# apple/foundationdb

Hardware: AMD Instinct MI355X
Metric: device-resident CRC32C GiB/s on 4 KiB page batches; % of HBM-read peak (higher is better)
Workload: dtype u8; 1 GPU; 1048576 x 4096 B pages, device-resident, fixed stride; pages=1048576, page_bytes=4096, seed=0, stride=4096

## Files before the change

foundationdb_amd/csrc/crc32c_device.h:

```cpp
#pragma once
#include <stdint.h>
#include <hip/hip_runtime.h>

#include <mutex>

namespace fdbcrc {

constexpr uint32_t kV7TabSlots = 64u;

struct DevTables {
	uint32_t slice[2][256];
	uint32_t block[8][16];
	uint32_t lane[64][8][16];
	uint32_t slice4[4][256];
	uint32_t inv_z[16][8][16];
	uint32_t pow2[64][8][16];
	uint32_t corr[4][16][8][16];
	uint32_t table_shift[8][16];
	uint32_t slotw[64][16][8][16];
	uint32_t carryw[64][16][8][16];
	uint32_t chunkpow[256][8][16];
	uint32_t bpow[4][256][8][16];
	uint32_t xinv64[65][8][16];
	uint32_t pow64[64][8][16];
	uint32_t pow1[64][8][16];
	uint32_t stride4[4][256];
	uint32_t lane_s[64][8][16];
};

void build_dev_tables(DevTables* t);

constexpr uint32_t kPageCtrWords = 32;

#ifndef FDBCRC_XCD_EVEN_W
#define FDBCRC_XCD_EVEN_W 33
#define FDBCRC_XCD_ODD_W 31
#endif
constexpr uint64_t kXcdEvenW = FDBCRC_XCD_EVEN_W, kXcdOddW = FDBCRC_XCD_ODD_W;
struct XcdRanges {
	uint64_t n, pe, po;
	__device__ __forceinline__ XcdRanges(uint64_t n_, uint64_t G) : n(n_) {
		const uint64_t ne = (G + 1) / 2, no = G / 2;
		const uint64_t den = ne * kXcdEvenW + no * kXcdOddW;
		const uint64_t unit = (n * 32 + den - 1) / den;
		pe = (unit * kXcdEvenW + 31) / 32;
		po = (unit * kXcdOddW + 31) / 32;
	}
	__device__ __forceinline__ void get(uint64_t b, uint64_t& g0, uint64_t& g1) const {
		const uint64_t s0 = ((b + 1) / 2) * pe + (b / 2) * po;
		const uint64_t e0 = s0 + ((b & 1) ? po : pe);
		g0 = s0 < n ? s0 : n;
		g1 = e0 < n ? e0 : n;
	}
};
__device__ __forceinline__ void xcd_range(uint64_t n, uint64_t b, uint64_t G, uint64_t& g0, uint64_t& g1) {
	XcdRanges(n, G).get(b, g0, g1);
}
int page_counters(hipStream_t stream, int num_cus, uint32_t** ctr);
constexpr uint64_t kAuxBytes = 256;
constexpr int kAuxPktFrames = 0;
constexpr int kAuxPageCtr = 8;
int stream_aux(hipStream_t stream, uint64_t** aux, std::unique_lock<std::mutex>* hold = nullptr);

int launch_pages(int blocks_per_page, const uint8_t* base, uint64_t stride, uint64_t count, uint32_t seed,
                 const uint32_t* seeds, uint32_t* out, const DevTables* tabs, int num_cus, hipStream_t stream);
int launch_pages_window(const uint8_t* pages, uint64_t stride, uint64_t count, uint32_t h, uint32_t t, uint32_t seed,
                        const uint32_t* seeds, uint32_t* out, const DevTables* tabs, int num_cus, hipStream_t stream);
int launch_pages_window_list(const uint8_t* pages, uint64_t stride, const uint32_t* idx, const uint64_t* d_count,
                             uint64_t max_count, uint32_t h, uint32_t t, uint32_t seed, uint32_t* out,
                             const DevTables* tabs, int num_cus, hipStream_t stream);
enum : int { kRouteBoth = 0, kRouteWindows = 1, kRouteBlocks = 2, kRouteExtent = 3 };
constexpr int kHstatNblk = 3, kHstatPacked = 4, kHstatXfail = 5;
constexpr uint64_t kXfailBackoff = 16;
inline int route_for_stats(const volatile uint64_t* s) {
	const uint64_t win = s[0], mid = s[1], large = s[2];
	const bool big = large != 0 && large >= win + mid;
	if (s[kHstatPacked] == 1 && s[kHstatXfail] == 0 && !big) return kRouteExtent;
	if (!big) return kRouteWindows;
	return win == 0 ? kRouteBlocks : kRouteBoth;
}
constexpr uint64_t kXMaxExtent = 1ull << 40;
#ifndef FDBX_GRAB_MIN
#define FDBX_GRAB_MIN 8
#endif
constexpr uint64_t kXGrabMin = FDBX_GRAB_MIN;
static_assert(kXGrabMin >= 8 && (kXGrabMin & (kXGrabMin - 1)) == 0, "grabs: a power of two of at least 8 blocks");
__host__ __device__ inline uint64_t x_gsz(uint64_t nblk, uint64_t capg) {
	uint64_t gsz = kXGrabMin;
	while (capg && (nblk + gsz - 1) / gsz > capg) gsz <<= 1;
	return gsz;
}
__host__ __device__ inline uint32_t x_log2(uint64_t v) {
	uint32_t l = 0;
	while ((1ull << l) < v) ++l;
	return l;
}
constexpr uint64_t kXGrabCap = 1ull << 18;
constexpr int kXStage = 8;
struct XState {
	uint32_t* xhdr;
	uint32_t* ps;
	uint32_t* pe;
	uint32_t* dummy;
	uint32_t* ragg;
	uint32_t* wq;
	uint32_t* gagg;
	uint64_t capg;
	uint32_t* ctr;
	uint32_t epoch;
};
uint64_t extent_state_bytes(uint64_t count, uint64_t capg, int num_cus);
void extent_state_carve(void* mem, uint64_t count, uint64_t capg, int num_cus, XState* x);
uint64_t varlen_workspace_bytes(uint64_t count, uint64_t nwave);
int launch_varlen(const uint8_t* base, const uint64_t* offsets, const uint64_t* lengths, uint64_t count, uint32_t seed,
                  const uint32_t* seeds, uint32_t* out, const DevTables* tabs, int num_cus, void* ws,
                  hipStream_t stream, int route = kRouteBoth, uint64_t* hstat = nullptr, uint32_t* err = nullptr,
                  const XState* xs = nullptr, uint32_t* bacc = nullptr, uint32_t* pctr = nullptr);
inline const uint64_t* varlen_refused_word(const void* ws) { return static_cast<const uint64_t*>(ws) + 6; }
int launch_fixed_general(const uint8_t* base, uint64_t stride, uint64_t length, uint64_t count, uint32_t seed,
                         const uint32_t* seeds, uint32_t* out, const DevTables* tabs, int num_cus, void* ws,
                         hipStream_t stream);
uint64_t varlen7_workspace_bytes(uint64_t count, uint64_t nwave);
int launch_varlen7(const uint8_t* base, const uint64_t* offsets, const uint64_t* lengths, uint64_t stride,
                   uint64_t length, uint64_t count, uint32_t seed, const uint32_t* seeds, uint32_t* out,
                   const DevTables* tabs, int num_cus, void* ws, hipStream_t stream, int route, uint64_t* hstat,
                   uint32_t* err = nullptr, const XState* xs = nullptr, uint32_t* bacc = nullptr,
                   uint32_t* pctr = nullptr);
int launch_extent(const uint8_t* base, const uint64_t* offsets, const uint64_t* lengths, uint64_t stride,
                  uint64_t length, uint64_t count, uint32_t seed, const uint32_t* seeds, uint32_t* out,
                  const DevTables* tabs, int num_cus, const XState& xs, uint64_t* hstat, hipStream_t stream,
                  int phase);
int launch_chain_fold(const uint64_t* starts, uint64_t nchains, const uint64_t* lengths, const uint32_t* segcrc,
                      uint32_t seed, const uint32_t* seeds, uint32_t* out, const DevTables* tabs, int num_cus,
                      hipStream_t stream);
struct BigEnt {
	uint64_t E;
	uint32_t s;
	uint32_t idx;
	uint32_t lot;
	uint32_t sd;
};
struct BigParams {
	const uint64_t* hdr;
	const BigEnt* ent;
	uint32_t* out;
	uint32_t* ctr;
	const DevTables* tabs;
	const uint8_t* base;
	const uint64_t* offsets;
	const uint64_t* lengths;
	uint64_t nbuf;
	uint32_t seed;
	const uint32_t* seeds;
	uint32_t* acc;
	BigEnt* priv;
	uint64_t* hstat;
	uint32_t* err;
};
constexpr uint64_t kNPMax = 6144;
constexpr uint64_t kNPAccBytes = 8 * kNPMax + 32;
int launch_bigblocks_np(const BigParams& P, int num_cus, hipStream_t stream);
constexpr uint64_t kBigMax = 1ull << 40;
int launch_bigblocks(const BigParams& P, int num_cus, hipStream_t stream);
int launch_fill_seeds(uint64_t count, uint32_t seed, const uint32_t* seeds, uint32_t* out, hipStream_t stream);

}
```

foundationdb_amd/csrc/crc32c_kernels.hip:

```cpp

#include <hip/hip_runtime.h>
#include <stdint.h>

#include <type_traits>

#include "crc32c_common.h"

#ifndef FDBCRC_PU
#define FDBCRC_PU 2
#endif

namespace fdbcrc {

template <int U, bool WINDOW, bool RAW = WINDOW>
__device__ __forceinline__ void unit_crc_b(const uint32_t* lds, int lane, uint32_t c4, uint32_t c_lane,
                                           Block (&u)[U], const uint32_t (&s)[U], uint32_t (&crc)[U],
                                           uint32_t h, uint32_t t) {
	if (WINDOW) {
#pragma unroll
		for (int j = 0; j < U; ++j) {
			const Masks mk = edge_masks(h, 16 - t, ~s[j]);
#pragma unroll
			for (int d = 0; d < 4; ++d) {
				const uint32_t m0 = lane == 0 ? mk.lm[d] : ~0u;
				const uint32_t x0 = lane == 0 ? mk.inj[d] : ((d == 0 && lane == 32) ? mk.spill : 0u);
				u[j].r[0][d] = (u[j].r[0][d] & m0) ^ x0;
				u[j].r[3][d] &= lane == 63 ? mk.tm[d] : ~0u;
			}
		}
	}
#pragma unroll
	for (int j = 0; j < U; ++j) unswizzle(u[j]);
	uint32_t x[U];
#pragma unroll
	for (int j = 0; j < U; ++j) x[j] = (!WINDOW && lane == 0) ? ~s[j] : 0u;
#pragma unroll
	for (int j = 0; j < U; ++j) x[j] ^= u[j].r[0][0];
#pragma unroll
	for (int w = 0; w < 16; ++w)
#pragma unroll
		for (int j = 0; j < U; ++j) x[j] = word_step4_next(lds, x[j], w < 15 ? u[j].r[(w + 1) >> 2][(w + 1) & 3] : 0u, c4);
#pragma unroll
	for (int j = 0; j < U; ++j) {
		const uint32_t r = wave_xor(mul_nibbles(lds, x[j], c_lane));
		crc[j] = RAW ? r : ~r;
	}
}

struct BlockS {
	uint32_t w[16];
};
typedef __attribute__((address_space(1))) const uint32_t g_u32k;
__device__ __forceinline__ void load_block_s(BlockS& b, const uint8_t* page, uint32_t lane4) {
	const uint8_t* p = page + lane4;
#pragma unroll
	for (int k = 0; k < 16; ++k) b.w[k] = __builtin_nontemporal_load((g_u32k*)reinterpret_cast<uintptr_t>(p + 256 * k));
}
template <int U, bool WINDOW, bool RAW = WINDOW>
__device__ __forceinline__ void unit_crc_s(const uint32_t* lds, int lane, uint32_t c4, uint32_t c_lane,
                                           BlockS (&u)[U], const uint32_t (&s)[U], uint32_t (&crc)[U],
                                           uint32_t h, uint32_t t) {
	uint32_t x[U];
	if (WINDOW) {
		const int d = (int)h - 4 * lane;
		const uint32_t keep0 = d <= 0 ? ~0u : (d >= 4 ? 0u : ~0u << (8 * d));
		const int cut = 256 - (int)t - 4 * lane;
		const uint32_t keep15 = cut >= 4 ? ~0u : (cut <= 0 ? 0u : ~0u >> (8 * (4 - cut)));
#pragma unroll
		for (int j = 0; j < U; ++j) {
			const uint32_t sd = ~s[j];
			const uint32_t inj = (d > -4 && d < 4) ? (d >= 0 ? sd << (8 * d) : sd >> (-8 * d)) : 0u;
			x[j] = (u[j].w[0] & keep0) ^ inj;
			u[j].w[15] &= keep15;
		}
	} else {
#pragma unroll
		for (int j = 0; j < U; ++j) x[j] = (lane == 0 ? ~s[j] : 0u) ^ u[j].w[0];
	}
#pragma unroll
	for (int w = 0; w < 16; ++w)
#pragma unroll
		for (int j = 0; j < U; ++j) x[j] = word_step4_next(lds, x[j], w < 15 ? u[j].w[w + 1] : 0u, c4);
#pragma unroll
	for (int j = 0; j < U; ++j) {
		const uint32_t r = wave_xor(mul_nibbles(lds, x[j], c_lane));
		crc[j] = RAW ? r : ~r;
	}
}

__device__ __forceinline__ uint32_t vmul_tab(const uint32_t (*tab)[16], uint32_t v) {
	typedef __attribute__((address_space(1))) const uint32_t g_u32;
	uint32_t r = 0;
#pragma unroll
	for (int n = 0; n < 8; ++n)
		r ^= *((g_u32*)reinterpret_cast<uintptr_t>(&tab[n][(v >> (4 * n)) & 15u]));
	return r;
}

#ifdef FDBCRC_BTIMES
__device__ uint64_t g_bt[16384][4];
__device__ uint64_t g_bt2[16384][4];
#define FDBCRC_BT2(k) \
	{ \
		const uint64_t tk = __builtin_amdgcn_s_memrealtime(); \
		const uint32_t wk = blockIdx.x * 16 + (threadIdx.x >> 6); \
		if ((threadIdx.x & 63) == 0) __hip_atomic_store(&g_bt2[wk][k], tk, __ATOMIC_RELAXED, __HIP_MEMORY_SCOPE_AGENT); \
	}
#else
#define FDBCRC_BT2(k)
#endif
#ifndef FDBCRC_STRIDED
#define FDBCRC_STRIDED 0
#endif
template <int U, bool WINDOW = false, bool LIST = false, bool PAIR = false, bool STRIDED = FDBCRC_STRIDED>
__global__ __launch_bounds__(1024) void k_pages4k(const uint8_t* __restrict__ base, uint64_t stride, uint64_t count,
                                                  uint32_t seed, const uint32_t* __restrict__ seeds,
                                                  uint32_t* __restrict__ out, const DevTables* __restrict__ tabs,
                                                  uint32_t* __restrict__ ctr, uint32_t h = 0, uint32_t t = 0,
                                                  const uint32_t* __restrict__ idx = nullptr,
                                                  const uint64_t* __restrict__ d_count = nullptr) {
	if (LIST) {
		count = *d_count;
		if (count == 0) return;
	}
	if (PAIR) count *= 2;
#ifdef FDBCRC_BTIMES
	const uint64_t pt0 = __builtin_amdgcn_s_memrealtime();
#endif
	constexpr uint32_t C = 2 * U;
	constexpr uint32_t F = 64 / C;
	static_assert(64 % C == 0, "a store group fills the wave's lanes");
	__shared__ uint32_t lds[kLdsBytesB / 4];
	const LaneCtx c = make_ctx();
	const uint32_t col4 = (c.lane & 31) * 4;
	const uint32_t c4 = col4 | 0x10000u;
	const uint32_t c_lane = (kS4LaneOff + (c.lane >> 5) * 0x4000) | col4;
	const uint32_t wpb = blockDim.x >> 6;
	const uint32_t wi = rdfirst(threadIdx.x >> 6);
	const uint64_t ngrab = (count + C - 1) / C;
	uint64_t g0, g1;
	xcd_range(ngrab, blockIdx.x, gridDim.x, g0, g1);
	uint32_t* const my_ctr = ctr + kPageCtrWords * blockIdx.x;
	const uint64_t last = count - 1;
	auto page = [&](uint64_t i) {
		const uint64_t j = i < count ? i : last;
		if (PAIR) return base + (j >> 1) * stride + (j & 1) * 4096;
		return base + (LIST ? (uint64_t)idx[j] : j) * stride;
	};
	typedef typename std::conditional<STRIDED, BlockS, Block>::type Blk;
	const uint32_t lane4 = 4u * (uint32_t)c.lane;
	auto load_u = [&](Blk (&u)[U], uint64_t i0) {
#pragma unroll
		for (int j = 0; j < U; ++j) {
			if constexpr (STRIDED)
				load_block_s(u[j], page(i0 + j), lane4);
			else
				load_block(u[j], page(i0 + j), c.ld_off);
		}
	};
	auto unit = [&](Blk (&u)[U], const uint32_t (&sd)[U], uint32_t (&crc)[U]) {
		if constexpr (STRIDED)
			unit_crc_s<U, WINDOW, WINDOW || PAIR>(lds, c.lane, c4, c_lane, u, sd, crc, h, t);
		else
			unit_crc_b<U, WINDOW, WINDOW || PAIR>(lds, c.lane, c4, c_lane, u, sd, crc, h, t);
	};
	auto clampg = [&](uint64_t g) { return g < g1 ? g : ngrab; };
	auto request = [&]() -> uint32_t {
		uint32_t r = 0;
		if (c.lane == 0) r = atomicAdd(my_ctr, 1u);
		return r;
	};
	auto seed_of = [&](uint64_t g) -> uint32_t {
		const uint64_t i = g * C + (uint64_t)(c.lane & (C - 1));
		const uint64_t j = i < count ? i : last;
		const uint32_t v = *(seeds ? seeds + (PAIR ? j >> 1 : j) : &tabs->slice4[0][0]);
		const uint32_t sd = seeds ? v : seed;
		return (PAIR && (c.lane & 1)) ? ~0u : sd;
	};
	uint64_t gA = clampg(g0 + wi), gB = ngrab;
	uint32_t sdA = seed_of(gA), sdB = 0;
	Blk u0[U], u1[U];
	load_u(u0, gA * C);
	if constexpr (STRIDED)
		fill_lds_src(lds, &tabs->stride4[0][0], &tabs->lane_s[0][0][0]);
	else
		fill_lds_b(lds, tabs);
	uint32_t mine = 0;
	uint64_t myi = ~0ull;
	uint32_t f = 0;
	constexpr uint32_t kDefer = 8;
	const bool defer = count < 0xFFFFFFFFull;
	uint32_t dm[kDefer], di[kDefer];
	uint32_t nd = 0;
	auto finish = [&](uint32_t m, uint64_t i) {
		if (WINDOW) m = ~(t ? vmul_tab(tabs->inv_z[t], m) : m);
		if (PAIR) {
			const uint32_t other = __builtin_amdgcn_update_dpp(0u, m, 0xB1, 0xF, 0xF, false);
			m = ~(vmul_tab(tabs->block, m) ^ other);
			if (i < count && !(c.lane & 1)) out[i >> 1] = m;
		} else if (i < count) {
			out[i] = m;
		}
	};
	auto flush_held = [&]() {
#pragma unroll
		for (uint32_t q = 0; q < kDefer; ++q)
			if (q < nd) finish(dm[q], di[q] == ~0u ? ~0ull : (uint64_t)di[q]);
		nd = 0;
	};
	auto store = [&]() {
		if (defer) {
#pragma unroll
			for (uint32_t q = 0; q < kDefer; ++q)
				if (q == nd) {
					dm[q] = mine;
					di[q] = myi < count ? (uint32_t)myi : ~0u;
				}
			if (++nd == kDefer) flush_held();
		} else {
			finish(mine, myi);
		}
		myi = ~0ull;
	};
	while (gA < ngrab) {
		const uint64_t first = gA * C;
		const uint32_t l0 = f * C;
		uint32_t sd[U], crc[U];
		const uint32_t req = request();
		load_u(u1, first + U);
		__builtin_amdgcn_sched_barrier(0);
#pragma unroll
		for (int j = 0; j < U; ++j) sd[j] = rdlane(sdA, j);
		unit(u0, sd, crc);
#pragma unroll
		for (int j = 0; j < U; ++j) mine = (uint32_t)c.lane == l0 + j ? crc[j] : mine;
		__builtin_amdgcn_sched_barrier(0);
		gB = clampg(g0 + wpb + rdlane(req, 0));
		sdB = seed_of(gB);
		load_u(u0, gB * C);
		__builtin_amdgcn_sched_barrier(0);
#pragma unroll
		for (int j = 0; j < U; ++j) sd[j] = rdlane(sdA, U + j);
		unit(u1, sd, crc);
#pragma unroll
		for (int j = 0; j < U; ++j) mine = (uint32_t)c.lane == l0 + U + j ? crc[j] : mine;
		__builtin_amdgcn_sched_barrier(0);
		const uint32_t k = (uint32_t)c.lane - l0;
		myi = k < C ? first + k : myi;
		gA = gB;
		sdA = sdB;
		if (++f == F) {
			store();
			f = 0;
		}
	}
	if (f) store();
	flush_held();
#ifdef FDBCRC_BTIMES
	if (c.lane == 0) {
		const uint32_t w = blockIdx.x * (blockDim.x >> 6) + (threadIdx.x >> 6);
		if (w < 16384) {
			g_bt[w][0] = pt0;
			g_bt[w][1] = __builtin_amdgcn_s_memrealtime();
			g_bt[w][2] = 0;
			g_bt[w][3] = 0;
		}
	}
#endif
	__builtin_amdgcn_s_waitcnt(0);
	__syncthreads();
	if (threadIdx.x == 0) *my_ctr = 0;
}

__device__ __forceinline__ void chunk_slot(uint32_t o, uint32_t& ln, uint32_t& ri) {
	ln = 32 * ((o >> 4) & 1) + 16 * ((o >> 5) & 1) + ((o >> 6) & 15);
	ri = ((o >> 11) & 1) | (((o >> 10) & 1) << 1);
}
typedef __attribute__((address_space(4))) const BigParams KBig;
__device__ __forceinline__ KBig* big_kargs() {
#if defined(__HIP_DEVICE_COMPILE__)
	KBig* kp = (KBig*)__builtin_amdgcn_kernarg_segment_ptr();
	asm volatile("" : "+s"(kp));
	return kp;
#else
	return nullptr;
#endif
}
struct NPGeo {
	uint32_t nb;
	bool refuse;
};
__device__ __forceinline__ NPGeo np_geo(uint64_t P0, uint64_t len) {
	NPGeo g;
	const uint64_t E = (P0 + len + 15) & ~uint64_t(15), A = P0 & ~uint64_t(15);
	const uint64_t span = E - A;
	g.refuse = len >= 16 && span >= kBigMax;
	g.nb = len >= 16 && !g.refuse ? (uint32_t)((span + 4095) >> 12) : 0u;
	return g;
}
__device__ __forceinline__ BigEnt np_entry(uint64_t P0, uint64_t len, uint32_t nb, uint32_t s, uint32_t idx,
                                           uint32_t seed) {
	const uint64_t E = (P0 + len + 15) & ~uint64_t(15), A = P0 & ~uint64_t(15);
	const uint32_t lo = (uint32_t)(4096ull * nb - (E - A));
	BigEnt e;
	e.E = E;
	e.s = s;
	e.idx = idx;
	e.lot = (lo >> 4) | ((uint32_t)(P0 & 15) << 8) | ((uint32_t)(E - (P0 + len)) << 12);
	e.sd = ~seed;
	return e;
}
struct NPStart {
	uint32_t count, nbig;
	uint32_t qa, qlim;
	uint32_t smallm;
	uint32_t m;
	bool refused;
};
__device__ __forceinline__ void lds_barrier() { asm volatile("s_waitcnt lgkmcnt(0)\n\ts_barrier" ::: "memory"); }
constexpr uint32_t kNPRing = 0;
constexpr uint32_t kNPScratch = 1024;
constexpr uint32_t kNPStats = 1088;
constexpr uint32_t kNPHand = 1200;
constexpr uint32_t kNPBlocks = 2048;
constexpr uint32_t kNPGeo = kNPBlocks + kNPMax;
static_assert(kNPGeo + 4 * kNPMax <= kLdsBytesB / 4, "prep-free start-up: its LDS scratch fits the table image");
template <uint32_t C>
__device__ NPStart np_start(const BigParams& P, uint32_t* lds, uint32_t ngrid) {
	typedef __attribute__((address_space(1))) const uint64_t g_u64;
	auto gl64 = [](const uint64_t* p) -> uint64_t { return *((g_u64*)reinterpret_cast<uintptr_t>(p)); };
	NPStart R;
	const uint32_t t = threadIdx.x, lane = t & 63, wv = t >> 6;
	const uint64_t n = P.nbuf;
	const uint32_t m = (uint32_t)((n + 1023) >> 10);
	const uint64_t i0 = (uint64_t)t * m;
	uint32_t* const nbl = lds + kNPBlocks;
	uint64_t* const sB = reinterpret_cast<uint64_t*>(lds + kNPScratch);
	uint32_t* const sN = lds + kNPScratch + 32;
	uint32_t* const sR = lds + kNPScratch + 48;
	uint64_t B = 0;
	uint32_t N = 0, smallm = 0;
	bool refuse = false;
	for (uint32_t j0 = 0; j0 < m; j0 += 8) {
		uint64_t o[8], l[8];
		uint32_t sd[8];
#pragma unroll
		for (uint32_t u = 0; u < 8; ++u) {
			const uint64_t ic = j0 + u < m && i0 + j0 + u < n ? i0 + j0 + u : 0;
			o[u] = gl64(P.offsets + ic);
			l[u] = gl64(P.lengths + ic);
			sd[u] = P.seeds ? P.seeds[ic] : P.seed;
		}
#pragma unroll
		for (uint32_t u = 0; u < 8; ++u) {
			if (j0 + u < m && i0 + j0 + u < n) {
				const uint64_t P0 = reinterpret_cast<uint64_t>(P.base) + o[u];
				const NPGeo g = np_geo(P0, l[u]);
				nbl[i0 + j0 + u] = g.nb;
				const BigEnt e = np_entry(P0, l[u], g.nb, 0u, 0u, sd[u]);
				*reinterpret_cast<u32x4*>(lds + kNPGeo + 4 * (uint32_t)(i0 + j0 + u)) =
				    u32x4{(uint32_t)e.E, (uint32_t)(e.E >> 32), e.lot, e.sd};
				B += g.nb;
				N += g.nb ? 1u : 0u;
				refuse |= g.refuse;
				smallm |= (g.nb == 0 && !g.refuse ? 1u : 0u) << (j0 + u);
			}
		}
	}
	FDBCRC_BT2(0)
	uint64_t Bi = B;
	uint32_t Ni = N;
#pragma unroll
	for (int d = 1; d < 64; d <<= 1) {
		const uint64_t vb = ((uint64_t)(uint32_t)__shfl_up((int)(uint32_t)(Bi >> 32), d) << 32) |
		                    (uint32_t)__shfl_up((int)(uint32_t)Bi, d);
		const uint32_t vn = (uint32_t)__shfl_up((int)Ni, d);
		if (lane >= (uint32_t)d) {
			Bi += vb;
			Ni += vn;
		}
	}
	const bool wref = __ballot(refuse) != 0;
	if (lane == 63) {
		sB[wv] = Bi;
		sN[wv] = Ni;
		sR[wv] = wref ? 1u : 0u;
	}
	__syncthreads();
	FDBCRC_BT2(1)
	constexpr uint32_t nw = 16;
	const uint32_t kl = lane & 15;
	uint64_t sb16 = sB[kl];
	uint32_t sn16 = sN[kl];
	const bool ref = __ballot(sR[kl] != 0) != 0;
#pragma unroll
	for (int d = 1; d < 16; d <<= 1) {
		const uint64_t vb = ((uint64_t)(uint32_t)__shfl_up((int)(uint32_t)(sb16 >> 32), d, 16) << 32) |
		                    (uint32_t)__shfl_up((int)(uint32_t)sb16, d, 16);
		const uint32_t vn = (uint32_t)__shfl_up((int)sn16, d, 16);
		if (kl >= (uint32_t)d) {
			sb16 += vb;
			sn16 += vn;
		}
	}
	const uint64_t Btot = rdlane64(sb16, 15);
	const uint32_t Ntot = rdlane(sn16, 15);
	const uint64_t Bex = Bi - B + (wv ? rdlane64(sb16, (int)wv - 1) : 0);
	const uint32_t Nex = Ni - N + (wv ? rdlane(sn16, (int)wv - 1) : 0u);
	R.refused = ref || Btot >= 0xFFFFFFFFull;
	R.count = R.refused ? 0u : (uint32_t)Btot;
	R.nbig = Ntot;
	R.smallm = smallm;
	R.m = m;
	R.qa = R.qlim = 0;
	const uint32_t ngrab = (uint32_t)(((uint64_t)R.count + C - 1) / C);
	const uint32_t per = (ngrab + ngrid - 1) / ngrid;
	const uint32_t g0 = blockIdx.x * per, g1 = g0 + per < ngrab ? g0 + per : ngrab;
	const uint64_t blo = (uint64_t)g0 * C;
	const uint64_t bhi = g1 * (uint64_t)C < R.count ? g1 * (uint64_t)C : R.count;
	BigEnt* const priv = P.priv + 2 * blockIdx.x;
	auto put = [&](uint32_t q, const BigEnt& e) {
		priv[q] = e;
		uint32_t* const r = lds + kNPRing + 6 * (q & 127u);
		r[0] = (uint32_t)e.E;
		r[1] = (uint32_t)(e.E >> 32);
		r[2] = e.s;
		r[3] = e.idx;
		r[4] = e.lot;
		r[5] = e.sd;
	};
	if (!R.refused && g0 < g1 && Bex < bhi && Bex + B > blo) {
		uint64_t sb = Bex;
		uint32_t q = Nex;
		for (uint32_t j = 0; j < m; ++j) {
			const uint64_t i = i0 + j;
			if (i >= n || sb >= bhi) break;
			const uint32_t nb = nbl[i];
			if (!nb) continue;
			if (sb + nb > blo) {
				const u32x4 gq = *reinterpret_cast<const u32x4*>(lds + kNPGeo + 4 * (uint32_t)i);
				BigEnt e;
				e.E = ((uint64_t)gq[1] << 32) | gq[0];
				e.s = (uint32_t)sb;
				e.idx = (uint32_t)i;
				e.lot = gq[2];
				e.sd = gq[3];
				put(q, e);
				if (sb <= blo) lds[kNPHand] = q;
				if (bhi <= sb + nb) {
					BigEnt z;
					z.E = 0;
					z.s = (uint32_t)(sb + nb);
					z.idx = ~0u;
					z.lot = 0;
					z.sd = 0;
					put(q + 1, z);
					lds[kNPHand + 1] = q + 1;
				}
			}
			sb += nb;
			++q;
		}
	}
	if (blockIdx.x == 0 && P.hstat && t < 256) {
		const uint64_t i = t;
		const bool ok = i < n;
		const uint64_t off = ok ? P.offsets[i] : 0, len = ok ? P.lengths[i] : 0;
		const bool nx = i + 1 < n;
		const uint64_t on = nx ? P.offsets[i + 1] : 0;
		const uint64_t P0 = reinterpret_cast<uint64_t>(P.base) + off;
		const uint64_t span = ok && len >= 16 ? ((P0 + len + 15) & ~uint64_t(15)) - (P0 & ~uint64_t(15)) : 0;
		const uint64_t e = off + len, gap = on - e;
		uint64_t c[4] = {span > 128 && span < 4096 ? len : 0, span >= 4096 && span < 16384 ? len : 0,
		                 span >= 16384 ? len : 0,
		                 (ok && nx && !(on >= e && gap < 4096 && gap <= (len > 256 ? len : 256))) ? 1u : 0u};
#pragma unroll
		for (int k = 0; k < 4; ++k)
			for (int o = 32; o > 0; o >>= 1)
				c[k] += ((uint64_t)(uint32_t)__shfl_xor((int)(uint32_t)(c[k] >> 32), o) << 32) |
				        (uint32_t)__shfl_xor((int)(uint32_t)c[k], o);
		uint64_t* const s64 = reinterpret_cast<uint64_t*>(lds + kNPStats);
		if (lane == 0)
#pragma unroll
			for (int k = 0; k < 4; ++k) s64[4 * wv + k] = c[k];
	}
	lds_barrier();
	FDBCRC_BT2(2)
	R.qa = rdfirst(lds[kNPHand]);
	R.qlim = rdfirst(lds[kNPHand + 1]);
	if (R.qlim - R.qa >= 64 && !R.refused && g0 < g1) {
		__builtin_amdgcn_s_waitcnt(0);
		__syncthreads();
	}
	if (blockIdx.x == 0 && t == 0 && P.hstat) {
		const uint64_t* const s64 = reinterpret_cast<const uint64_t*>(lds + kNPStats);
		uint64_t* const park = reinterpret_cast<uint64_t*>(P.acc + 2 * kNPMax);
		for (int k = 0; k < 4; ++k) park[k] = s64[k] + s64[4 + k] + s64[8 + k] + s64[12 + k];
	}
	return R;
}

template <int U, bool NP>
__global__ __launch_bounds__(1024) void k_bigblocks(BigParams P) {
#ifdef FDBCRC_BTIMES
	const uint64_t bt0 = __builtin_amdgcn_s_memrealtime();
#endif
	typedef __attribute__((address_space(1))) const uint64_t g_u64;
	typedef __attribute__((address_space(1))) const uint32_t g_u32;
	auto gl32 = [](const uint32_t* p) -> uint32_t { return *((g_u32*)reinterpret_cast<uintptr_t>(p)); };
	auto gl64 = [](const uint64_t* p) -> uint64_t { return *((g_u64*)reinterpret_cast<uintptr_t>(p)); };
	const uint32_t ngrid = gridDim.x;
	asm volatile("" ::"s"(ngrid));
	FillRegs fill;
	fill_issue_1024(fill, P.tabs);
	constexpr uint32_t C = 2 * U;
	constexpr uint32_t F = 64 / C;
	__shared__ uint32_t lds[kLdsBytesB / 4];
	NPStart S;
	uint32_t count, nbig;
	if (NP) {
		S = np_start<C>(P, lds, ngrid);
		if (S.refused) {
			if (blockIdx.x == 0 && threadIdx.x == 0 && P.err) *P.err = 1u;
			return;
		}
		count = S.count;
		nbig = S.nbig;
	} else {
		count = (uint32_t)rdfirst64(gl64(P.hdr + 2));
		if (count == 0) return;
		nbig = (uint32_t)rdfirst64(gl64(P.hdr + 3));
	}
	const DevTables* __restrict__ T = P.tabs;
	const LaneCtx c = make_ctx();
	const uint32_t lane = (uint32_t)c.lane;
	const uint32_t col4 = (lane & 31) * 4;
	const uint32_t c4 = col4 | 0x10000u;
	const uint32_t c_lane = (kS4LaneOff + (lane >> 5) * 0x4000) | col4;
	constexpr uint32_t wpb = 16;
	const uint32_t wi = rdfirst(threadIdx.x >> 6);
	const uint32_t ngrab = (uint32_t)(((uint64_t)count + C - 1) / C);
	const uint32_t per = (ngrab + ngrid - 1) / ngrid;
	const uint32_t g0 = blockIdx.x * per;
	const uint32_t g1 = g0 + per < ngrab ? g0 + per : ngrab;
	uint32_t* const my_ctr = P.ctr + kPageCtrWords * blockIdx.x;
	const uint32_t last = (uint32_t)(count - 1);

	uint32_t wj = 0;
	uint32_t ws = 0, wI = 0, wL = 0, wS = 0, wend = 0;
	uint64_t wE = 0;
	auto ent = [&](uint32_t q) -> BigEnt {
		const uint64_t* w = reinterpret_cast<const uint64_t*>(NP ? big_kargs()->priv + 2 * blockIdx.x + q : P.ent + q);
		uint64_t w0, w1, w2;
		if (NP) {
			w0 = __hip_atomic_load(w, __ATOMIC_RELAXED, __HIP_MEMORY_SCOPE_AGENT);
			w1 = __hip_atomic_load(w + 1, __ATOMIC_RELAXED, __HIP_MEMORY_SCOPE_AGENT);
			w2 = __hip_atomic_load(w + 2, __ATOMIC_RELAXED, __HIP_MEMORY_SCOPE_AGENT);
		} else {
			w0 = gl64(w);
			w1 = gl64(w + 1);
			w2 = gl64(w + 2);
		}
		BigEnt e;
		e.E = w0;
		e.s = (uint32_t)w1;
		e.idx = (uint32_t)(w1 >> 32);
		e.lot = (uint32_t)w2;
		e.sd = (uint32_t)(w2 >> 32);
		return e;
	};
	auto ent_s = [&](uint32_t q) -> uint32_t {
		if (NP)
			return __hip_atomic_load(&big_kargs()->priv[2 * blockIdx.x + q].s, __ATOMIC_RELAXED,
			                         __HIP_MEMORY_SCOPE_AGENT);
		return gl32(&P.ent[q].s);
	};
	const uint32_t qtop = NP ? S.qlim : nbig - 1;
	auto load_window = [&](uint32_t j0) {
		const uint32_t q = j0 + lane;
		const uint32_t qc = q <= qtop ? q : qtop;
		const BigEnt e = ent(qc);
		const uint32_t s = e.s;
		wE = e.E;
		wI = e.idx;
		wL = e.lot;
		wS = e.sd;
		if (NP) {
			const uint32_t qe = (uint64_t)j0 + 64 <= qtop ? j0 + 64 : qtop;
			const uint32_t se = ent_s(qe);
			ws = q <= qtop ? s : ~0u;
			wend = (uint64_t)j0 + 64 <= qtop ? rdfirst(se) : count;
		} else {
			const uint32_t qe = (uint64_t)j0 + 64 < nbig ? j0 + 64 : nbig - 1;
			const uint32_t se = ent_s(qe);
			ws = q < nbig ? s : (q == nbig ? count : ~0u);
			wend = (uint64_t)j0 + 64 < nbig ? rdfirst(se) : count;
		}
		wj = j0;
	};
	auto find = [&](uint32_t b) -> uint32_t {
		uint32_t q0 = 0, n = nbig;
		for (;;) {
			if (n <= 64) {
				const uint32_t v = ent_s(q0 + (lane < n ? lane : 0));
				const bool le = lane < n && v <= b;
				return q0 + (uint32_t)__builtin_popcountll(__ballot(le)) - 1;
			}
			const uint32_t stp = (n + 255) >> 8;
			uint32_t v[4];
#pragma unroll
			for (uint32_t u = 0; u < 4; ++u) {
				const uint64_t k = (4 * (uint64_t)lane + u) * stp;
				v[u] = ent_s(q0 + (uint32_t)(k < n ? k : 0));
			}
			uint32_t cnt = 0;
#pragma unroll
			for (uint32_t u = 0; u < 4; ++u) {
				const uint64_t k = (4 * (uint64_t)lane + u) * stp;
				cnt += (uint32_t)__builtin_popcountll(__ballot(k < n && v[u] <= b));
			}
			if (stp == 1) return q0 + cnt - 1;
			q0 += (cnt - 1) * stp;
			n = n - (cnt - 1) * stp < stp ? n - (cnt - 1) * stp : stp;
		}
	};

	struct Meta {
		uint32_t alo, ahi, kt, ek, sd, idx, nbt;
	};
	auto rd = [](uint32_t v, uint32_t j) { return rdlane(v, (int)j); };
	auto pick = [&](Meta& M, uint32_t b0) {
		const uint32_t j = lane & (C - 1);
		int e = 0;
#pragma unroll
		for (uint32_t t = 0; t < C; ++t) {
			const uint32_t bt = b0 + t <= last ? b0 + t : last;
			const int et = (int)__builtin_popcountll(__ballot(ws <= bt)) - 1;
			e = j == t ? et : e;
		}
		const uint32_t b = b0 + j <= last ? b0 + j : last;
		const int src = e << 2;
		const uint32_t se = (uint32_t)__builtin_amdgcn_ds_bpermute(src, (int)ws);
		const uint32_t sn1 = (uint32_t)__builtin_amdgcn_ds_bpermute(src + 4, (int)ws);
		const uint32_t sn = e < 63 ? sn1 : wend;
		const uint32_t lot = (uint32_t)__builtin_amdgcn_ds_bpermute(src, (int)wL);
		const uint32_t eEl = (uint32_t)__builtin_amdgcn_ds_bpermute(src, (int)(uint32_t)wE);
		const uint32_t eEh = (uint32_t)__builtin_amdgcn_ds_bpermute(src, (int)(uint32_t)(wE >> 32));
		const uint32_t sdv = (uint32_t)__builtin_amdgcn_ds_bpermute(src, (int)wS);
		const uint32_t ixv = (uint32_t)__builtin_amdgcn_ds_bpermute(src, (int)wI);
		const uint32_t m = b - se;
		const uint32_t k = sn - se - 1 - m;
		const uint64_t a = (((uint64_t)eEh << 32) | eEl) - 4096ull * (k + 1);
		M.alo = (uint32_t)a;
		M.ahi = (uint32_t)(a >> 32);
		M.kt = k | ((lot >> 12) << 28);
		M.ek = m == 0 ? lot & 0xFFFu : 0u;
		M.sd = m == 0 ? sdv : 0u;
		M.idx = b0 + j <= last ? ixv : ~0u;
		M.nbt = sn - se;
	};
	auto meta_of = [&](uint32_t g, Meta& M) {
		const uint64_t bf = (uint64_t)g * C;
		if (bf >= count) {
			const uint64_t a0 = rdlane64(wE, 0) - 4096;
			const uint32_t lo16 = rdlane(ws, 1) - rdlane(ws, 0) == 1 ? rdlane(wL, 0) & 0xFFu : 0u;
			M.alo = (uint32_t)a0;
			M.ahi = (uint32_t)(a0 >> 32);
			M.kt = 0;
			M.ek = lo16;
			M.sd = 0;
			M.idx = ~0u;
			M.nbt = 0;
			return;
		}
		const uint32_t b0 = (uint32_t)bf;
		const uint32_t bl = bf + C - 1 < count ? b0 + C - 1 : last;
		if (bl >= wend) {
			do {
				const uint32_t adv = b0 < wend ? (uint32_t)__builtin_popcountll(__ballot(ws <= b0)) - 1u : 64u;
				load_window(wj + adv);
			} while (bl >= wend);
			pick(M, b0);
		} else {
			pick(M, b0);
		}
	};
	auto load_u = [&](Block (&u)[U], const Meta& M, uint32_t j0) {
#pragma unroll
		for (uint32_t j = 0; j < U; ++j) {
			const uint8_t* blk = reinterpret_cast<const uint8_t*>(((uint64_t)rd(M.ahi, j0 + j) << 32) | rd(M.alo, j0 + j));
			const uint32_t lo = (rd(M.ek, j0 + j) & 0xFFu) << 4;
#pragma unroll
			for (int k = 0; k < 4; ++k) {
				uint32_t off = c.ld_off + 2048u * (k & 1) + 1024u * (k >> 1);
				off = off > lo ? off : lo;
				u[j].r[k] = ld16(blk + off);
			}
		}
	};
	auto crc_u = [&](Block (&u)[U], const Meta& M, uint32_t j0, uint32_t (&crc)[U]) {
		uint32_t spill[U];
#pragma unroll
		for (uint32_t j = 0; j < U; ++j) {
			const uint32_t kt = rd(M.kt, j0 + j), ek = rd(M.ek, j0 + j), sd = rd(M.sd, j0 + j);
			spill[j] = 0;
			if (ek | sd) {
				const uint32_t lo = (ek & 0xFFu) << 4, k0 = ek >> 8;
#pragma unroll
				for (int k = 0; k < 4; ++k) {
					const bool z = c.ld_off + 2048u * (k & 1) + 1024u * (k >> 1) < lo;
#pragma unroll
					for (int d = 0; d < 4; ++d) u[j].r[k][d] = z ? 0u : u[j].r[k][d];
				}
				const Masks mk = edge_masks(k0, 16u, sd);
				uint32_t ln, ri;
				chunk_slot(lo, ln, ri);
				const bool lead_lane = lane == ln;
#pragma unroll
				for (uint32_t k = 0; k < 4; ++k) {
					const bool on = lead_lane && k == ri;
#pragma unroll
					for (int d = 0; d < 4; ++d) u[j].r[k][d] = on ? ((u[j].r[k][d] & mk.lm[d]) ^ mk.inj[d]) : u[j].r[k][d];
				}
				const bool in_blk = lo + 16 < 4096;
				chunk_slot((lo + 16) & 4095u, ln, ri);
				const bool sp_lane = in_blk && lane == ln;
#pragma unroll
				for (uint32_t k = 0; k < 4; ++k) u[j].r[k][0] ^= (sp_lane && k == ri) ? mk.spill : 0u;
				spill[j] = in_blk ? 0u : mk.spill;
			}
			const uint32_t t = kt >> 28;
			if ((kt & 0xFFFFFFFu) == 0 && t) {
				const Masks mt = edge_masks(0u, 16u - t, 0u);
#pragma unroll
				for (int d = 0; d < 4; ++d) u[j].r[3][d] &= lane == 63 ? mt.tm[d] : ~0u;
			}
		}
		uint32_t sd[U];
#pragma unroll
		for (uint32_t j = 0; j < U; ++j) sd[j] = ~0u;
		unit_crc_b<U, false, true>(lds, c.lane, c4, c_lane, u, sd, crc, 0, 0);
#pragma unroll
		for (uint32_t j = 0; j < U; ++j) crc[j] ^= spill[j];
	};

	uint32_t mine = 0, mkt = 0, midx = ~0u, mnbt = 0;
	auto store = [&]() {
		const uint32_t k = mkt & 0xFFFFFFFu, t = mkt >> 28;
		uint32_t w = vmul_tab(T->bpow[0][k & 255u], mine);
		if (__ballot(k >= (1u << 8))) w = vmul_tab(T->bpow[1][(k >> 8) & 255u], w);
		if (__ballot(k >= (1u << 16))) w = vmul_tab(T->bpow[2][(k >> 16) & 255u], w);
		if (__ballot(k >= (1u << 24))) w = vmul_tab(T->bpow[3][k >> 24], w);
		w = vmul_tab(T->inv_z[t], w);
		uint32_t nrun = 1;
#pragma unroll
		for (int d = 1; d < 64; d <<= 1) {
			const uint32_t y = (uint32_t)__shfl_up((int)w, d);
			const uint32_t yi = (uint32_t)__shfl_up((int)midx, d);
			const uint32_t yn = NP ? (uint32_t)__shfl_up((int)nrun, d) : 0u;
			if ((int)lane >= d && yi == midx) {
				w ^= y;
				nrun += yn;
			}
		}
		const uint32_t ni = (uint32_t)__shfl_down((int)midx, 1);
		if (midx != ~0u && (lane == 63 || ni != midx)) {
			if (!NP) {
				atomicXor(P.out + midx, w);
			} else {
				uint32_t* const acc = big_kargs()->acc + midx;
				uint32_t* const cnt = acc + kNPMax;
				const uint32_t old = atomicXor(acc, w);
				asm volatile("" ::"v"(old));
				const uint32_t done = atomicAdd(cnt, nrun) + nrun;
				if (done == mnbt) {
					const uint32_t v = atomicExch(acc, 0u);
					atomicExch(cnt, 0u);
					big_kargs()->out[midx] = ~v;
				}

			}
		}
		midx = ~0u;
	};

	auto clampg = [&](uint32_t g) { return g < g1 ? g : ngrab; };
	auto request = [&]() -> uint32_t {
		uint32_t r = 0;
		if (lane == 0) r = atomicAdd(my_ctr, 1u);
		return r;
	};
	uint32_t gA = clampg(g0 + wi);
	const bool run = !NP || (count > 0 && g0 < g1);
	if (!NP) {
		if (wi == 0) {
			const uint32_t q = find(g0 * C < count ? (uint32_t)(g0 * C) : last);
			if (lane < wpb) lds[kS4Off / 4 + 256 * lane] = q;
		}
		__syncthreads();
		load_window(rdfirst(lds[kS4Off / 4 + 256 * wi]));
	} else if (run) {
		if (S.qlim - S.qa < 64) {
			const uint32_t q = S.qa + lane, qc = q <= S.qlim ? q : S.qlim;
			const uint32_t* const r = lds + kNPRing + 6 * (qc & 127u);
			wE = ((uint64_t)r[1] << 32) | r[0];
			ws = q <= S.qlim ? r[2] : ~0u;
			wI = r[3];
			wL = r[4];
			wS = r[5];
			wend = count;
			wj = S.qa;
		} else {
			load_window(S.qa);
		}

	}
	Meta MA, MB;
	Block u0[U], u1[U];
	if (run) {
		meta_of(gA, MA);
		load_u(u0, MA, 0);
	}
	FDBCRC_BT2(3)
	if (NP) lds_barrier();
	fill_commit_1024(fill, lds);
#ifdef FDBCRC_BTIMES
	const uint64_t bt1 = __builtin_amdgcn_s_memrealtime();
#endif
	uint32_t f = 0;
	auto step = [&](Meta& X, Meta& Y) {
		const uint32_t l0 = f * C;
		uint32_t crc[U];
		const uint32_t req = request();
		load_u(u1, X, U);
		__builtin_amdgcn_sched_barrier(0);
		crc_u(u0, X, 0, crc);
#pragma unroll
		for (uint32_t j = 0; j < U; ++j) mine = lane == l0 + j ? crc[j] : mine;
		{
			const bool mine_grab = lane - l0 < C;
			const int src = (int)(((lane - l0) & (C - 1)) << 2);
			const uint32_t kt = (uint32_t)__builtin_amdgcn_ds_bpermute(src, (int)X.kt);
			const uint32_t ix = (uint32_t)__builtin_amdgcn_ds_bpermute(src, (int)X.idx);
			mkt = mine_grab ? kt : mkt;
			midx = mine_grab ? ix : midx;
			if (NP) {
				const uint32_t nt = (uint32_t)__builtin_amdgcn_ds_bpermute(src, (int)X.nbt);
				mnbt = mine_grab ? nt : mnbt;
			}
		}
		__builtin_amdgcn_sched_barrier(0);
		const uint32_t gB = clampg(g0 + wpb + rdlane(req, 0));
		meta_of(gB, Y);
		load_u(u0, Y, 0);
		__builtin_amdgcn_sched_barrier(0);
		crc_u(u1, X, U, crc);
#pragma unroll
		for (uint32_t j = 0; j < U; ++j) mine = lane == l0 + U + j ? crc[j] : mine;
		__builtin_amdgcn_sched_barrier(0);
		gA = gB;
		if (++f == F) {
			store();
			f = 0;
		}
	};
	if (run) {
		while (gA < ngrab) {
			step(MA, MB);
			if (gA >= ngrab) break;
			step(MB, MA);
		}
		if (f) store();
	}
#ifdef FDBCRC_BTIMES
	const uint64_t bt2 = __builtin_amdgcn_s_memrealtime();
#endif
	if (NP) {
		KBig* const K = big_kargs();
		const uint64_t i0 = (uint64_t)threadIdx.x * S.m;
		for (uint32_t msk = S.smallm; msk;) {
			const uint32_t j = (uint32_t)__builtin_ctz(msk);
			msk &= msk - 1;
			const uint64_t i = i0 + j;
			if (i % ngrid != blockIdx.x) continue;
			const uint8_t* b = K->base + K->offsets[i];
			const uint32_t len = (uint32_t)K->lengths[i];
			uint32_t r = ~(K->seeds ? K->seeds[i] : K->seed);
			for (uint32_t k = 0; k < len; ++k)
				r = (r >> 8) ^ lds_rd(lds, (0x10000u | (((r ^ ld1(b + k)) & 255u) << 8) | col4) + 128);
			K->out[i] = ~r;
		}
		uint64_t* const hs = K->hstat;
		if (blockIdx.x == 0 && threadIdx.x == 0 && hs) {
			const uint64_t* const park = reinterpret_cast<const uint64_t*>(K->acc + 2 * kNPMax);
			for (int k = 0; k < 3; ++k) hs[k] = park[k];
			hs[kHstatPacked] = park[3] ? 0 : 1;
			if (hs[kHstatXfail] > 0 && hs[kHstatXfail] <= kXfailBackoff) --hs[kHstatXfail];
		}
	}
#ifdef FDBCRC_BTIMES
	if (lane == 0) {
		const uint32_t w = blockIdx.x * wpb + wi;
		g_bt[w][0] = bt0;
		g_bt[w][1] = bt2;
		g_bt[w][2] = bt1;
		g_bt[w][3] = __builtin_amdgcn_s_memrealtime();
	}
#endif
	__builtin_amdgcn_s_waitcnt(0);
	__syncthreads();
	if (threadIdx.x == 0) *my_ctr = 0;
}

int launch_bigblocks(const BigParams& P, int num_cus, hipStream_t stream) {
	k_bigblocks<FDBCRC_PU, false><<<(unsigned)num_cus, 1024, 0, stream>>>(P);
	return 0;
}

int launch_bigblocks_np(const BigParams& P, int num_cus, hipStream_t stream) {
	if (P.nbuf == 0 || P.nbuf > kNPMax || !P.offsets || !P.lengths || !P.acc || !P.priv || !P.ctr) return -1;
	k_bigblocks<FDBCRC_PU, true><<<(unsigned)num_cus, 1024, 0, stream>>>(P);
	return 0;
}

static unsigned page_grid(uint64_t pages, int num_cus) {
	const uint64_t grabs = (pages + 2 * FDBCRC_PU - 1) / (2 * FDBCRC_PU);
	uint64_t grid = (grabs + 15) / 16;
	if (grid > (uint64_t)num_cus) grid = num_cus;
	return grid ? (unsigned)grid : 1u;
}

int launch_pages(int blocks_per_page, const uint8_t* base, uint64_t stride, uint64_t count, uint32_t seed,
                 const uint32_t* seeds, uint32_t* out, const DevTables* tabs, int num_cus, hipStream_t stream) {
	if (count == 0) return 0;
	uint32_t* ctr;
	if (page_counters(stream, num_cus, &ctr)) return -1;
	switch (blocks_per_page) {
		case 1:
			k_pages4k<FDBCRC_PU><<<page_grid(count, num_cus), 1024, 0, stream>>>(base, stride, count, seed, seeds, out,
			                                                                      tabs, ctr);
			break;
		case 2:
			k_pages4k<FDBCRC_PU, false, false, true><<<page_grid(2 * count, num_cus), 1024, 0, stream>>>(
			    base, stride, count, seed, seeds, out, tabs, ctr);
			break;
		default: return -1;
	}
	return 0;
}

int launch_pages_window(const uint8_t* pages, uint64_t stride, uint64_t count, uint32_t h, uint32_t t, uint32_t seed,
                        const uint32_t* seeds, uint32_t* out, const DevTables* tabs, int num_cus, hipStream_t stream) {
	if (count == 0) return 0;
	uint32_t* ctr;
	if (page_counters(stream, num_cus, &ctr)) return -1;
	k_pages4k<FDBCRC_PU, true><<<page_grid(count, num_cus), 1024, 0, stream>>>(pages, stride, count, seed, seeds, out,
	                                                                          tabs, ctr, h, t);
	return 0;
}

int launch_pages_window_list(const uint8_t* pages, uint64_t stride, const uint32_t* idx, const uint64_t* d_count,
                             uint64_t max_count, uint32_t h, uint32_t t, uint32_t seed, uint32_t* out,
                             const DevTables* tabs, int num_cus, hipStream_t stream) {
	if (max_count == 0) return 0;
	uint32_t* ctr;
	if (page_counters(stream, num_cus, &ctr)) return -1;
	k_pages4k<FDBCRC_PU, true, true><<<page_grid(max_count, num_cus), 1024, 0, stream>>>(
	    pages, stride, max_count, seed, nullptr, out, tabs, ctr, h, t, idx, d_count);
	return 0;
}

#ifdef FDBCRC_DEBUG
__global__ void k_dbg_set_pages(unsigned long long lo, unsigned long long hi) {
	g_dbg[0] = lo; g_dbg[1] = hi;
	for (int k = 2; k < 8; ++k) g_dbg[k] = 0;
}
__global__ void k_dbg_get_pages(unsigned long long* out) {
	for (int k = 0; k < 8; ++k) out[k] = g_dbg[k];
}
void dbg_set_pages(uint64_t lo, uint64_t hi) { k_dbg_set_pages<<<1, 1>>>(lo, hi); }
void dbg_get_pages(uint64_t* d_out8) { k_dbg_get_pages<<<1, 1>>>(reinterpret_cast<unsigned long long*>(d_out8)); }
#endif

__global__ void k_fill_seeds(uint64_t count, uint32_t seed, const uint32_t* __restrict__ seeds,
                             uint32_t* __restrict__ out) {
	for (uint64_t i = (uint64_t)blockIdx.x * blockDim.x + threadIdx.x; i < count; i += (uint64_t)gridDim.x * blockDim.x)
		out[i] = seeds ? seeds[i] : seed;
}

int launch_fill_seeds(uint64_t count, uint32_t seed, const uint32_t* seeds, uint32_t* out, hipStream_t stream) {
	uint64_t grid = (count + 255) / 256;
	if (grid > 4096) grid = 4096;
	k_fill_seeds<<<(unsigned)grid, 256, 0, stream>>>(count, seed, seeds, out);
	return 0;
}

}

#ifdef FDBCRC_BTIMES
extern "C" int fdbcrc_debug_btimes(void* host, uint64_t nwave) {
	return (int)hipMemcpyFromSymbol(host, HIP_SYMBOL(fdbcrc::g_bt), nwave * 32, 0, hipMemcpyDeviceToHost);
}
extern "C" int fdbcrc_debug_btimes2(void* host, uint64_t nwave) {
	return (int)hipMemcpyFromSymbol(host, HIP_SYMBOL(fdbcrc::g_bt2), nwave * 32, 0, hipMemcpyDeviceToHost);
}
#endif
```

foundationdb_amd/csrc/crc32c_tables.cpp:

```cpp
#include <string.h>

#include "crc32c_device.h"
#include "crc32c_math.h"

namespace fdbcrc {

void build_dev_tables(DevTables* t) {
	memset(t, 0, sizeof(*t));
	for (uint32_t b = 0; b < 256; ++b) {
		const uint32_t t0 = byte_step(b);
		t->slice[1][b] = t0;
		t->slice[0][b] = (t0 >> 8) ^ byte_step(t0 & 0xffu);
	}
	for (uint32_t b = 0; b < 256; ++b) t->slice4[3][b] = byte_step(b);
	for (int k = 2; k >= 0; --k)
		for (uint32_t b = 0; b < 256; ++b)
			t->slice4[k][b] = (t->slice4[k + 1][b] >> 8) ^ byte_step(t->slice4[k + 1][b] & 0xffu);
	mul_tables_nibble(xpow8(4096), t->block);
	for (int l = 0; l < 64; ++l) mul_tables_nibble(xpow8(64u * (63 - l)), t->lane[l]);
	for (int z = 0; z < 16; ++z) mul_tables_nibble(xpow8_inv(z), t->inv_z[z]);
	for (int q = 0; q < 4; ++q)
		for (int z = 0; z < 16; ++z) mul_tables_nibble(xpow8_inv(z + 1024u * (3 - q)), t->corr[q][z]);
	mul_tables_nibble(xpow8(1024u * kV7TabSlots), t->table_shift);
	for (int d = 0; d < 64; ++d)
		for (int z = 0; z < 16; ++z) {
			const int64_t e = 1024 * (int64_t)(d - 3) - z;
			mul_tables_nibble(e >= 0 ? xpow8((uint64_t)e) : xpow8_inv((uint64_t)-e), t->slotw[d][z]);
			mul_tables_nibble(xpow8(1024u * (d + 1) - z), t->carryw[d][z]);
		}
	for (int c = 0; c < 256; ++c) mul_tables_nibble(xpow8(16u * (255 - c)), t->chunkpow[c]);
	for (int i = 0; i < 4; ++i)
		for (int j = 0; j < 256; ++j) mul_tables_nibble(xpow8((4096ull * j) << (8 * i)), t->bpow[i][j]);
	for (int j = 0; j <= 64; ++j) mul_tables_nibble(xpow8_inv(64u * j), t->xinv64[j]);
	for (int c = 0; c < 64; ++c) {
		mul_tables_nibble(xpow8(64u * c), t->pow64[c]);
		mul_tables_nibble(xpow8(c), t->pow1[c]);
	}
	mul_tables_byte(xpow8(256), t->stride4);
	for (int l = 0; l < 64; ++l) mul_tables_nibble(xpow8_inv(4u * l), t->lane_s[l]);
	for (int m = 0; m < 64; ++m) {
		uint32_t c = kOne >> 8;
		for (int k = 0; k < m; ++k) c = gf2_mul(c, c);
		mul_tables_nibble(c, t->pow2[m]);
	}
}

}
```

Measured before the change: 6273 GiB/s.

## Replace strided/block page CRC path with unswizzled word-step unit and seedless specialization

Removes the experimental strided-load variant and replaces the per-page unit with a new routine that unswizzles the standard block layout and runs word-step updates over 15 words, using a new per-lane combine table with a 4-byte shift folded in. Adds a SEEDS template flag so the no-seed path never loads per-page seeds, computing seed injection from a register. Moves the final inversion into the store. The aim is fewer table lookups and seed loads per page, at the cost of extra unswizzle shuffles and more kernel instantiations.

```diff
diff --git a/foundationdb_amd/csrc/crc32c_device.h b/foundationdb_amd/csrc/crc32c_device.h
--- a/foundationdb_amd/csrc/crc32c_device.h
+++ b/foundationdb_amd/csrc/crc32c_device.h
@@ -24,8 +24,7 @@
 	uint32_t xinv64[65][8][16];
 	uint32_t pow64[64][8][16];
 	uint32_t pow1[64][8][16];
-	uint32_t stride4[4][256];
-	uint32_t lane_s[64][8][16];
+	uint32_t lane32[64][8][16];
 };
 
 void build_dev_tables(DevTables* t);
diff --git a/foundationdb_amd/csrc/crc32c_kernels.hip b/foundationdb_amd/csrc/crc32c_kernels.hip
--- a/foundationdb_amd/csrc/crc32c_kernels.hip
+++ b/foundationdb_amd/csrc/crc32c_kernels.hip
@@ -1,8 +1,6 @@
 
 #include <hip/hip_runtime.h>
 #include <stdint.h>
-
-#include <type_traits>
 
 #include "crc32c_common.h"
 
@@ -47,45 +45,34 @@
 	}
 }
 
-struct BlockS {
-	uint32_t w[16];
-};
-typedef __attribute__((address_space(1))) const uint32_t g_u32k;
-__device__ __forceinline__ void load_block_s(BlockS& b, const uint8_t* page, uint32_t lane4) {
-	const uint8_t* p = page + lane4;
-#pragma unroll
-	for (int k = 0; k < 16; ++k) b.w[k] = __builtin_nontemporal_load((g_u32k*)reinterpret_cast<uintptr_t>(p + 256 * k));
-}
-template <int U, bool WINDOW, bool RAW = WINDOW>
-__device__ __forceinline__ void unit_crc_s(const uint32_t* lds, int lane, uint32_t c4, uint32_t c_lane,
-                                           BlockS (&u)[U], const uint32_t (&s)[U], uint32_t (&crc)[U],
-                                           uint32_t h, uint32_t t) {
+template <int U, bool WINDOW>
+__device__ __forceinline__ void unit_crc_p(const uint32_t* lds, int lane, uint32_t c4, uint32_t c_lane,
+                                           Block (&u)[U], const uint32_t (&s)[U], const uint32_t (&sx)[U],
+                                           uint32_t (&crc)[U], uint32_t h, uint32_t t) {
+	if (WINDOW) {
+#pragma unroll
+		for (int j = 0; j < U; ++j) {
+			const Masks mk = edge_masks(h, 16 - t, ~s[j]);
+#pragma unroll
+			for (int d = 0; d < 4; ++d) {
+				const uint32_t m0 = lane == 0 ? mk.lm[d] : ~0u;
+				const uint32_t x0 = lane == 0 ? mk.inj[d] : ((d == 0 && lane == 32) ? mk.spill : 0u);
+				u[j].r[0][d] = (u[j].r[0][d] & m0) ^ x0;
+				u[j].r[3][d] &= lane == 63 ? mk.tm[d] : ~0u;
+			}
+		}
+	}
+#pragma unroll
+	for (int j = 0; j < U; ++j) unswizzle(u[j]);
 	uint32_t x[U];
-	if (WINDOW) {
-		const int d = (int)h - 4 * lane;
-		const uint32_t keep0 = d <= 0 ? ~0u : (d >= 4 ? 0u : ~0u << (8 * d));
-		const int cut = 256 - (int)t - 4 * lane;
-		const uint32_t keep15 = cut >= 4 ? ~0u : (cut <= 0 ? 0u : ~0u >> (8 * (4 - cut)));
-#pragma unroll
-		for (int j = 0; j < U; ++j) {
-			const uint32_t sd = ~s[j];
-			const uint32_t inj = (d > -4 && d < 4) ? (d >= 0 ? sd << (8 * d) : sd >> (-8 * d)) : 0u;
-			x[j] = (u[j].w[0] & keep0) ^ inj;
-			u[j].w[15] &= keep15;
-		}
-	} else {
-#pragma unroll
-		for (int j = 0; j < U; ++j) x[j] = (lane == 0 ? ~s[j] : 0u) ^ u[j].w[0];
-	}
-#pragma unroll
-	for (int w = 0; w < 16; ++w)
-#pragma unroll
-		for (int j = 0; j < U; ++j) x[j] = word_step4_next(lds, x[j], w < 15 ? u[j].w[w + 1] : 0u, c4);
-#pragma unroll
-	for (int j = 0; j < U; ++j) {
-		const uint32_t r = wave_xor(mul_nibbles(lds, x[j], c_lane));
-		crc[j] = RAW ? r : ~r;
-	}
+#pragma unroll
+	for (int j = 0; j < U; ++j) x[j] = WINDOW ? u[j].r[0][0] : u[j].r[0][0] ^ sx[j];
+#pragma unroll
+	for (int w = 0; w < 15; ++w)
+#pragma unroll
+		for (int j = 0; j < U; ++j) x[j] = word_step4_next(lds, x[j], u[j].r[(w + 1) >> 2][(w + 1) & 3], c4);
+#pragma unroll
+	for (int j = 0; j < U; ++j) crc[j] = wave_xor(mul_nibbles(lds, x[j], c_lane));
 }
 
 __device__ __forceinline__ uint32_t vmul_tab(const uint32_t (*tab)[16], uint32_t v) {
@@ -109,10 +96,7 @@
 #else
 #define FDBCRC_BT2(k)
 #endif
-#ifndef FDBCRC_STRIDED
-#define FDBCRC_STRIDED 0
-#endif
-template <int U, bool WINDOW = false, bool LIST = false, bool PAIR = false, bool STRIDED = FDBCRC_STRIDED>
+template <int U, bool WINDOW = false, bool LIST = false, bool PAIR = false, bool SEEDS = false>
 __global__ __launch_bounds__(1024) void k_pages4k(const uint8_t* __restrict__ base, uint64_t stride, uint64_t count,
                                                   uint32_t seed, const uint32_t* __restrict__ seeds,
                                                   uint32_t* __restrict__ out, const DevTables* __restrict__ tabs,
@@ -147,22 +131,9 @@
 		if (PAIR) return base + (j >> 1) * stride + (j & 1) * 4096;
 		return base + (LIST ? (uint64_t)idx[j] : j) * stride;
 	};
-	typedef typename std::conditional<STRIDED, BlockS, Block>::type Blk;
-	const uint32_t lane4 = 4u * (uint32_t)c.lane;
-	auto load_u = [&](Blk (&u)[U], uint64_t i0) {
-#pragma unroll
-		for (int j = 0; j < U; ++j) {
-			if constexpr (STRIDED)
-				load_block_s(u[j], page(i0 + j), lane4);
-			else
-				load_block(u[j], page(i0 + j), c.ld_off);
-		}
-	};
-	auto unit = [&](Blk (&u)[U], const uint32_t (&sd)[U], uint32_t (&crc)[U]) {
-		if constexpr (STRIDED)
-			unit_crc_s<U, WINDOW, WINDOW || PAIR>(lds, c.lane, c4, c_lane, u, sd, crc, h, t);
-		else
-			unit_crc_b<U, WINDOW, WINDOW || PAIR>(lds, c.lane, c4, c_lane, u, sd, crc, h, t);
+	auto load_u = [&](Block (&u)[U], uint64_t i0) {
+#pragma unroll
+		for (int j = 0; j < U; ++j) load_block(u[j], page(i0 + j), c.ld_off);
 	};
 	auto clampg = [&](uint64_t g) { return g < g1 ? g : ngrab; };
 	auto request = [&]() -> uint32_t {
@@ -171,20 +142,34 @@
 		return r;
 	};
 	auto seed_of = [&](uint64_t g) -> uint32_t {
+		if constexpr (!SEEDS) return 0u;
 		const uint64_t i = g * C + (uint64_t)(c.lane & (C - 1));
 		const uint64_t j = i < count ? i : last;
-		const uint32_t v = *(seeds ? seeds + (PAIR ? j >> 1 : j) : &tabs->slice4[0][0]);
-		const uint32_t sd = seeds ? v : seed;
+		const uint32_t sd = seeds[PAIR ? j >> 1 : j];
 		return (PAIR && (c.lane & 1)) ? ~0u : sd;
+	};
+	const uint32_t sx_one = c.lane == 0 ? ~seed : 0u;
+	auto seeds_u = [&](uint32_t sdv, uint32_t j0, uint32_t (&s)[U], uint32_t (&sx)[U]) {
+#pragma unroll
+		for (uint32_t j = 0; j < U; ++j) {
+			if constexpr (SEEDS) {
+				s[j] = rdlane(sdv, (int)(j0 + j));
+				sx[j] = c.lane == 0 ? ~s[j] : 0u;
+			} else {
+				const bool second = PAIR && ((j0 + j) & 1);
+				s[j] = second ? ~0u : seed;
+				sx[j] = second ? 0u : sx_one;
+			}
+		}
+	};
+	auto unit = [&](Block (&u)[U], const uint32_t (&s)[U], const uint32_t (&sx)[U], uint32_t (&crc)[U]) {
+		unit_crc_p<U, WINDOW>(lds, c.lane, c4, c_lane, u, s, sx, crc, h, t);
 	};
 	uint64_t gA = clampg(g0 + wi), gB = ngrab;
 	uint32_t sdA = seed_of(gA), sdB = 0;
-	Blk u0[U], u1[U];
+	Block u0[U], u1[U];
 	load_u(u0, gA * C);
-	if constexpr (STRIDED)
-		fill_lds_src(lds, &tabs->stride4[0][0], &tabs->lane_s[0][0][0]);
-	else
-		fill_lds_b(lds, tabs);
+	fill_lds_src(lds, &tabs->slice4[0][0], &tabs->lane32[0][0][0]);
 	uint32_t mine = 0;
 	uint64_t myi = ~0ull;
 	uint32_t f = 0;
@@ -193,13 +178,13 @@
 	uint32_t dm[kDefer], di[kDefer];
 	uint32_t nd = 0;
 	auto finish = [&](uint32_t m, uint64_t i) {
-		if (WINDOW) m = ~(t ? vmul_tab(tabs->inv_z[t], m) : m);
+		if (WINDOW) m = t ? vmul_tab(tabs->inv_z[t], m) : m;
 		if (PAIR) {
 			const uint32_t other = __builtin_amdgcn_update_dpp(0u, m, 0xB1, 0xF, 0xF, false);
 			m = ~(vmul_tab(tabs->block, m) ^ other);
 			if (i < count && !(c.lane & 1)) out[i >> 1] = m;
 		} else if (i < count) {
-			out[i] = m;
+			out[i] = ~m;
 		}
 	};
 	auto flush_held = [&]() {
@@ -225,13 +210,12 @@
 	while (gA < ngrab) {
 		const uint64_t first = gA * C;
 		const uint32_t l0 = f * C;
-		uint32_t sd[U], crc[U];
+		uint32_t s[U], sx[U], crc[U];
 		const uint32_t req = request();
 		load_u(u1, first + U);
 		__builtin_amdgcn_sched_barrier(0);
-#pragma unroll
-		for (int j = 0; j < U; ++j) sd[j] = rdlane(sdA, j);
-		unit(u0, sd, crc);
+		seeds_u(sdA, 0, s, sx);
+		unit(u0, s, sx, crc);
 #pragma unroll
 		for (int j = 0; j < U; ++j) mine = (uint32_t)c.lane == l0 + j ? crc[j] : mine;
 		__builtin_amdgcn_sched_barrier(0);
@@ -239,9 +223,8 @@
 		sdB = seed_of(gB);
 		load_u(u0, gB * C);
 		__builtin_amdgcn_sched_barrier(0);
-#pragma unroll
-		for (int j = 0; j < U; ++j) sd[j] = rdlane(sdA, U + j);
-		unit(u1, sd, crc);
+		seeds_u(sdA, U, s, sx);
+		unit(u1, s, sx, crc);
 #pragma unroll
 		for (int j = 0; j < U; ++j) mine = (uint32_t)c.lane == l0 + U + j ? crc[j] : mine;
 		__builtin_amdgcn_sched_barrier(0);
@@ -937,12 +920,20 @@
 	if (page_counters(stream, num_cus, &ctr)) return -1;
 	switch (blocks_per_page) {
 		case 1:
-			k_pages4k<FDBCRC_PU><<<page_grid(count, num_cus), 1024, 0, stream>>>(base, stride, count, seed, seeds, out,
-			                                                                      tabs, ctr);
+			if (seeds)
+				k_pages4k<FDBCRC_PU, false, false, false, true><<<page_grid(count, num_cus), 1024, 0, stream>>>(
+				    base, stride, count, seed, seeds, out, tabs, ctr);
+			else
+				k_pages4k<FDBCRC_PU><<<page_grid(count, num_cus), 1024, 0, stream>>>(base, stride, count, seed, nullptr,
+				                                                                      out, tabs, ctr);
 			break;
 		case 2:
-			k_pages4k<FDBCRC_PU, false, false, true><<<page_grid(2 * count, num_cus), 1024, 0, stream>>>(
-			    base, stride, count, seed, seeds, out, tabs, ctr);
+			if (seeds)
+				k_pages4k<FDBCRC_PU, false, false, true, true><<<page_grid(2 * count, num_cus), 1024, 0, stream>>>(
+				    base, stride, count, seed, seeds, out, tabs, ctr);
+			else
+				k_pages4k<FDBCRC_PU, false, false, true><<<page_grid(2 * count, num_cus), 1024, 0, stream>>>(
+				    base, stride, count, seed, nullptr, out, tabs, ctr);
 			break;
 		default: return -1;
 	}
@@ -954,8 +945,12 @@
 	if (count == 0) return 0;
 	uint32_t* ctr;
 	if (page_counters(stream, num_cus, &ctr)) return -1;
-	k_pages4k<FDBCRC_PU, true><<<page_grid(count, num_cus), 1024, 0, stream>>>(pages, stride, count, seed, seeds, out,
-	                                                                          tabs, ctr, h, t);
+	if (seeds)
+		k_pages4k<FDBCRC_PU, true, false, false, true><<<page_grid(count, num_cus), 1024, 0, stream>>>(
+		    pages, stride, count, seed, seeds, out, tabs, ctr, h, t);
+	else
+		k_pages4k<FDBCRC_PU, true><<<page_grid(count, num_cus), 1024, 0, stream>>>(pages, stride, count, seed, nullptr,
+		                                                                          out, tabs, ctr, h, t);
 	return 0;
 }
 
diff --git a/foundationdb_amd/csrc/crc32c_tables.cpp b/foundationdb_amd/csrc/crc32c_tables.cpp
--- a/foundationdb_amd/csrc/crc32c_tables.cpp
+++ b/foundationdb_amd/csrc/crc32c_tables.cpp
@@ -36,8 +36,7 @@
 		mul_tables_nibble(xpow8(64u * c), t->pow64[c]);
 		mul_tables_nibble(xpow8(c), t->pow1[c]);
 	}
-	mul_tables_byte(xpow8(256), t->stride4);
-	for (int l = 0; l < 64; ++l) mul_tables_nibble(xpow8_inv(4u * l), t->lane_s[l]);
+	for (int l = 0; l < 64; ++l) mul_tables_nibble(xpow8(64u * (63 - l) + 4), t->lane32[l]);
 	for (int m = 0; m < 64; ++m) {
 		uint32_t c = kOne >> 8;
 		for (int k = 0; k < m; ++k) c = gf2_mul(c, c);
```

After: 6287 GiB/s, median of 6. No clear change (+0.2%).
